# Nablax/Path-Tracer-CUDA-OpenGL

Measured on AMD Instinct MI355X. Metric: Mray/s + ms/frame, bunny-in-Cornell 1920×1080 @1024spp, 1/2/4/8 MI355X, higher is better.
Workload: dtype f32

## Files before the change

### path-tracer-cuda-opengl_amd/csrc/pt_device.hip

```cpp
#include <hip/hip_runtime.h>

#include <algorithm>
#include <array>
#include <atomic>
#include <chrono>
#include <cfloat>
#include <cmath>
#include <cstdio>
#include <cstdlib>
#include <cstring>
#include <limits>
#include <type_traits>
#include <memory>
#include <string>
#include <vector>

#include "../host/pt_error.hpp"
#include "../host/pt_host.hpp"
#include "../host/pt_inst_dev.hpp"
#include "../host/pt_wide8.hpp"
#include "../host/pt_wide_dev.hpp"
#include "pt.h"
#include "pt_math.hpp"

// ... 259 lines not shown
    float b1 = dot3(s1, s) * inv;
    float b2 = dot3(s2, d) * inv;
    if (b1 >= 1.0f || b1 <= 0.0f || b2 >= 1.0f || b2 <= 0.0f || b1 + b2 >= 1.0f || t <= tmin)
        return -1.0f;
    return t;
}

__device__ __forceinline__ SlabHit refLeafBox(const Prim& q, bool sphere, float3 o, float3 inv, float tmin, float tmax) {
    float mn[3], mx[3];
    if (sphere) {
        const float r = fabsf(q.p1.x);
        mn[0] = q.p0.x - r; mn[1] = q.p0.y - r; mn[2] = q.p0.z - r;
        mx[0] = q.p0.x + r; mx[1] = q.p0.y + r; mx[2] = q.p0.z + r;
    } else {
        mn[0] = fminf(fminf(q.p0.x, q.p1.x), q.p2.x);
        mn[1] = fminf(fminf(q.p0.y, q.p1.y), q.p2.y);
        mn[2] = fminf(fminf(q.p0.z, q.p1.z), q.p2.z);
        mx[0] = fmaxf(fmaxf(q.p0.x, q.p1.x), q.p2.x);
        mx[1] = fmaxf(fmaxf(q.p0.y, q.p1.y), q.p2.y);
        mx[2] = fmaxf(fmaxf(q.p0.z, q.p1.z), q.p2.z);
    }
    return slabPair(v2f{mn[0], mx[0]}, v2f{mn[1], mx[1]}, v2f{mn[2], mx[2]}, o, inv, tmin, tmax);
}

template <bool SPH>
__device__ __forceinline__ void wideTest(const Prim& q, float3 o, float3 d, float3 inv, float tmin, float& closest,
                                         int& best, float& bestLo, bool leafBoxes, bool& redo, uint32_t keyHi = 0u) {
    const bool sph = SPH && __float_as_uint(q.p2.w) != 0u;
    const float t = primHitAny(q, sph, o, d, tmin);
    if (t >= 0.0f) {
        const int k = (int)(keyHi | __float_as_uint(q.p0.w));
        const bool none = best < 0, bSph = SPH && (best & (int)kSphereBit) != 0;
        const int bk = SPH ? best & (int)kPrimMask : best;
        const bool tie = sph ? (none || !bSph || k > bk) : (!none && !bSph && k < bk);
        redo = redo || (t >= closest && t < bestLo);
        if (t < closest || (t == closest && tie)) {
            bool take = true;
            float lo = -__builtin_inff();
            if (leafBoxes) {
                const SlabHit b = refLeafBox(q, sph, o, inv, tmin, __builtin_inff());
                take = b.hit && !(closest < b.lo);
                redo = redo || (b.hit && closest < b.lo);
                lo = t < b.lo ? b.lo : lo;
            }
            if (take) {
                closest = t;
                best = k | (sph ? (int)kSphereBit : 0);
                bestLo = lo;
            }
        }
    }
}

__device__ __forceinline__ void wideTestTri(const Prim& q, float3 o, float3 d, float tmin, float& closest, int& best,
                                            float& t2) {
    const float t = primHitAny(q, false, o, d, tmin);
    if (t >= 0.0f) {
        const int k = (int)__float_as_uint(q.p0.w);
        const bool better = t < closest || (t == closest && k < best);
        t2 = __builtin_amdgcn_fmed3f(t, closest, t2);
        closest = better ? t : closest;
        best = better ? k : best;
    }
}
__device__ __forceinline__ bool deferredRedo(float4 xy, float2 z, float3 o, float3 inv, float closest, float t2) {
    const SlabHit b = slabPair(v2f{xy.x, xy.y}, v2f{xy.z, xy.w}, v2f{z.x, z.y}, o, inv, 0.001f, __builtin_inff());
    return !b.hit || (closest < b.lo && t2 < b.lo);
}

template <bool MIX = false>
__device__ __forceinline__ uint32_t wideHits(uint4 n0, uint4 n1, uint4 n2, uint4 n3, uint4 n4, float3 o, float3 inv,
                                             uint32_t oct, float tmin, float tmax) {
    constexpr uint32_t kMixExp = MIX ? 24u : 0u;
    const float ax = __uint_as_float(((n0.w & 0xffu) + kMixExp) << 23) * inv.x;
    const float ay = __uint_as_float((((n0.w >> 8) & 0xffu) + kMixExp) << 23) * inv.y;
    const float az = __uint_as_float((((n0.w >> 16) & 0xffu) + kMixExp) << 23) * inv.z;
    const float bx = (__uint_as_float(n0.x) - o.x) * inv.x;
    const float by = (__uint_as_float(n0.y) - o.y) * inv.y;
    const float bz = (__uint_as_float(n0.z) - o.z) * inv.z;
    const bool sx = (oct & 1u) != 0, sy = (oct & 2u) != 0, sz = (oct & 4u) != 0;
    const uint32_t nearX[2] = {sx ? n2.z : n2.x, sx ? n2.w : n2.y}, farX[2] = {sx ? n2.x : n2.z, sx ? n2.y : n2.w};
    const uint32_t nearY[2] = {sy ? n3.z : n3.x, sy ? n3.w : n3.y}, farY[2] = {sy ? n3.x : n3.z, sy ? n3.y : n3.w};
    const uint32_t nearZ[2] = {sz ? n4.z : n4.x, sz ? n4.w : n4.y}, farZ[2] = {sz ? n4.x : n4.z, sz ? n4.y : n4.w};
    const uint32_t oct2 = oct | shlOpaque<8>(oct);
    const uint32_t oct4 = oct2 | (oct2 << 16);
    uint32_t hits = 0u;
#pragma unroll
    for (int h = 0; h < 2; h++) {
        const uint32_t meta4 = h ? n1.w : n1.z;
        const uint32_t inner4 = (meta4 & (meta4 << 1)) & 0x10101010u;
        const uint32_t inner1 = inner4 >> 4;
        const uint32_t innerMask4 = shlOpaque<3>(inner1) - inner1;
        const uint32_t bitIndex4 = (meta4 ^ (oct4 & innerMask4)) & 0x1f1f1f1fu;
        const uint32_t childBits4 = (meta4 >> 5) & 0x07070707u;
#pragma unroll
        for (int j = 0; j < 4; j++) {
            float tnx, tny, tnz, tfx, tfy, tfz;
            if constexpr (MIX) {
                const bool hi = (j & 2) != 0;
                const uint32_t px = hi ? planePairHi(nearX[h]) : planePairLo(nearX[h]);
                const uint32_t py = hi ? planePairHi(nearY[h]) : planePairLo(nearY[h]);
                const uint32_t pz = hi ? planePairHi(nearZ[h]) : planePairLo(nearZ[h]);
                const uint32_t qx = hi ? planePairHi(farX[h]) : planePairLo(farX[h]);
                const uint32_t qy = hi ? planePairHi(farY[h]) : planePairLo(farY[h]);
                const uint32_t qz = hi ? planePairHi(farZ[h]) : planePairLo(farZ[h]);
                if (j & 1) {
                    tnx = fmaMixHi(px, ax, bx); tny = fmaMixHi(py, ay, by); tnz = fmaMixHi(pz, az, bz);
                    tfx = fmaMixHi(qx, ax, bx); tfy = fmaMixHi(qy, ay, by); tfz = fmaMixHi(qz, az, bz);
                } else {
                    tnx = fmaMixLo(px, ax, bx); tny = fmaMixLo(py, ay, by); tnz = fmaMixLo(pz, az, bz);
                    tfx = fmaMixLo(qx, ax, bx); tfy = fmaMixLo(qy, ay, by); tfz = fmaMixLo(qz, az, bz);
                }
            } else {
                tnx = __builtin_fmaf((float)((nearX[h] >> (8 * j)) & 0xffu), ax, bx);
                tny = __builtin_fmaf((float)((nearY[h] >> (8 * j)) & 0xffu), ay, by);
                tnz = __builtin_fmaf((float)((nearZ[h] >> (8 * j)) & 0xffu), az, bz);
// ... 737 lines not shown
        closest = __builtin_inff();                                                               \
        best = -1;                                                                                \
        sp = 0;                                                                                   \
        qn = 0;                                                                                   \
        if constexpr (CRITK) pxRays++;                                                            \
        if constexpr (WIDE) {                 \
            inv = f3(rcpRN(d.x), rcpRN(d.y), rcpRN(d.z));                                         \
            const uint32_t oc_ = (inv.x < 0.0f ? 1u : 0u) | (inv.y < 0.0f ? 2u : 0u) | (inv.z < 0.0f ? 4u : 0u); \
            oct = oc_;                                                                            \
            tg = 0u;                                                                              \
                    \
            bestLo = INST || kargs()->S.hasSpheres ? -__builtin_inff() : __builtin_inff();         \
            ng = S.nprims > 0 ? (1u << oc_) : 0u;                                                 \
                 \
            if (!INST && ((kargs()->camFar && depthLeft + 1 == kargs()->max_depth) ||              \
                          (PT_WIDE_MIX && mixUnsafe(inv, kargs()->S.mixLim)))) {                   \
                ng = 0u;             \
                oct |= 8u;      \
            }                                                                                     \
            if (INST && kargs()->camFar && depthLeft + 1 == kargs()->max_depth) {                  \
                     \
                const auto& K_ = *kargs();                                                        \
                (void)instEntry(K_.S.cx, K_.S.cy, K_.S.cz, K_.S.ext, o, d, inv);                   \
            }                                                                                     \
            if (CRITK && crit) PT_CRIT_TRACE();                                                    \
        } else if (S.nprims <= 1) {                                                               \
            node = -1;                                                                            \
            if (S.nprims == 1) {        \
                const float t1 = primHitT(loadPrim(S, 0), __float_as_uint(S.prims[2].w) != 0, o, d, \
                                          0.001f, closest);                                       \
                if (t1 >= 0.0f) { closest = t1; best = 0; }                                       \
            }                                                                                     \
        } else {                                                                                  \
            inv = f3(rcpRN(d.x), rcpRN(d.y), rcpRN(d.z));                                         \
            node = 0;                                                                             \
        }                                                                                         \
    } while (0)
#define PT_CRIT_TRACE()                                                                             \
    do {                                                                                          \
        const bool lb_ = S.nprims > 1;                                                            \
        const bool sph_ = kargs()->S.hasSpheres != 0;                                             \
        bool redo_ = false;                                                                       \
        for (;;) {                                                                                \
            while (tg) {                                                                          \
                const uint32_t k_ = tgBase + (uint32_t)__builtin_ctz(tg);                         \
                tg &= tg - 1u;                                                                    \
                const float4* w_ = reinterpret_cast<const float4*>(reinterpret_cast<const char*>(S.wprims) + mul48(k_)); \
                const Prim q_{w_[0], w_[1], w_[2]};                                               \
                const bool isS_ = __float_as_uint(q_.p2.w) != 0u;                                 \
                sTris += (uint32_t)__popcll(__ballot(!isS_));                                     \
                sSph += (uint32_t)__popcll(__ballot(isS_));                                       \
                if (sph_) wideTest<true>(q_, o, d, inv, 0.001f, closest, best, bestLo, lb_, redo_, 0u); \
                else if (INST) wideTest<false>(q_, o, d, inv, 0.001f, closest, best, bestLo, lb_, redo_, 0u); \
                else wideTestTri(q_, o, d, 0.001f, closest, best, bestLo);    \
            }                                                                                     \
            if ((ng & 0xffu) == 0u) {                                                             \
                if (sp == 0) break;                                                               \
                sp--;                                                                             \
                ng = my[sp * kWave];                                                              \
            }                                                                                     \
            const uint32_t bit_ = (uint32_t)__builtin_ctz(ng & 0xffu);                            \
            const uint32_t child_ = (ng >> 8) + (bit_ ^ (oct & 7u));                              \
            ng &= ~(1u << bit_);                                                                  \
            if (ng & 0xffu) { my[sp * kWave] = ng; sp++; }    \
            sVisits += (uint32_t)__popcll(__ballot(true));                                        \
            const uint32_t off_ = mul80(child_);                                                  \
            const uint4 n0_ = __builtin_bit_cast(uint4, __builtin_amdgcn_raw_buffer_load_b128(nodeRsrc, off_, 0, 0)); \
            const uint4 n1_ = __builtin_bit_cast(uint4, __builtin_amdgcn_raw_buffer_load_b128(nodeRsrc, off_ + 16u, 0, 0)); \
            const uint4 n2_ = __builtin_bit_cast(uint4, __builtin_amdgcn_raw_buffer_load_b128(nodeRsrc, off_ + 32u, 0, 0)); \
            const uint4 n3_ = __builtin_bit_cast(uint4, __builtin_amdgcn_raw_buffer_load_b128(nodeRsrc, off_ + 48u, 0, 0)); \
            const uint4 n4_ = __builtin_bit_cast(uint4, __builtin_amdgcn_raw_buffer_load_b128(nodeRsrc, off_ + 64u, 0, 0)); \
            const uint32_t h_ = wideHits<PT_WIDE_MIX != 0>(n0_, n1_, n2_, n3_, n4_, o, inv, oct & 7u, 0.001f, closest); \
            ng = (n1_.x << 8) | (h_ >> 24);                                                      \
            tgBase = n1_.y;                                                                       \
            tg = h_ & 0xffffffu;                                                                  \
        }                                                                                         \
        if (redo_) oct |= 8u;              \
    } while (0)
#define PT_TAKE_TASKS(got)                                                                          \
    do {                                                                                          \
        const auto& Q_ = *kargs();                                                                \
        for (;;) {                                                                                \
            const uint64_t m_ = needTaskM;                                                        \
            if (m_ == 0) break;                                                                   \
            if (poolLeft == 0u) {  \
                const int leader_ = __ffsll((unsigned long long)m_) - 1;                          \
                          \
                const uint32_t grab_ = (uint32_t)kTaskPool;                                       \
                uint32_t b_ = 0;                                                                  \
                if (lane == leader_) b_ = atomicAdd(Q_.taskCounter, grab_);                       \
                poolBase = __builtin_amdgcn_readfirstlane((uint32_t)__shfl((int)b_, leader_));    \
                poolLeft = grab_;                                                                 \
            }                                                                                     \
              \
            const uint32_t base_ = poolBase;                                                      \
            const uint32_t take_ = min((uint32_t)__popcll(m_), poolLeft);                         \
            poolBase += take_;                                                                    \
            poolLeft -= take_;                                                                    \
            const uint32_t g0_ = base_ >> 6, off_ = base_ & 63u;                                  \
            const uint32_t slotA_ = Q_.nblocksShift >= 0 ? g0_ >> Q_.nblocksShift : g0_ / (uint32_t)Q_.ngroups; \
            const uint32_t blkA_ = g0_ - slotA_ * (uint32_t)Q_.ngroups;                           \
            const bool wrap_ = blkA_ + 1u == (uint32_t)Q_.ngroups;                                  \
            const uint32_t slotB_ = wrap_ ? slotA_ + 1u : slotA_, blkB_ = wrap_ ? 0u : blkA_ + 1u; \
            const uint32_t nslots_ = (uint32_t)Q_.ntiles;                                          \
             \
                                                    \
            const uint32_t xyA_ = slotA_ < nslots_ ? ((KU32)Q_.tileXY)[__builtin_amdgcn_readfirstlane(slotA_)] : 0u; \
// ... 267 lines not shown
                        sp++;
                    }
                    node = (int)rref;
                } else if (il) {
                    node = (int)lref;
                } else if (sp > 0) {
                    sp--;
                    node = (LS == STACK || sp < LS)
                               ? (int)my[sp * kWave]
                               : (int)P.stackSpill[((size_t)blockIdx.x * kWave + lane) * (STACK - LS) + (sp - LS)];
                } else {
                    node = -1;
                }
            }
        }
        if (kind == 1) {
            bool tested = false, sph = false;
            PT_DIAG_ADD(itL, 1u);
            if constexpr (WIDE) {
                PT_DIAG_ADD(sPops, (uint32_t)nL);
                uint32_t k0 = 0u, k1 = 0u;
                const bool h0 = laneOf(mL);
                if (h0) k0 = tgBase + (uint32_t)__builtin_ctz(tg);
                tg &= tg - 1u;
                const uint64_t m1 = __ballot((int)tg > 0);
                const bool h1 = laneOf(m1);
                if (h1) k1 = tgBase + (uint32_t)__builtin_ctz(tg);
                tg &= tg - 1u;
                const float4* w0 = reinterpret_cast<const float4*>(reinterpret_cast<const char*>(S.wprims) + mul48(k0));
                const float4* w1 = reinterpret_cast<const float4*>(reinterpret_cast<const char*>(S.wprims) + mul48(k1));
                const Prim q0{w0[0], w0[1], w0[2]}, q1{w1[0], w1[1], w1[2]};
                bool redo = false;
#ifdef PT_DIAG
                {
                    sHalf += (unsigned long long)__popcll(__ballot(h0 && !h1));
                    const bool pk = !INST && (oct & 64u) != 0u;
                    sParkT += (unsigned long long)(__popcll(__ballot(pk && h0)) + __popcll(__ballot(pk && h1)));
                }
#endif
                const bool lb = !INST && S.nprims > 1;
                const uint32_t kh = INST ? (oct >> 8) << kargs()->S.gBits : 0u;
                if (kargs()->S.hasSpheres) {
                    if (h0) wideTest<true>(q0, o, d, inv, 0.001f, closest, best, bestLo, lb, redo, kh);
                    if (h1) wideTest<true>(q1, o, d, inv, 0.001f, closest, best, bestLo, lb, redo, kh);
                    const uint64_t s0 = mL & __ballot(__float_as_uint(q0.p2.w) != 0u);
                    const uint64_t s1 = m1 & __ballot(__float_as_uint(q1.p2.w) != 0u);
                    sTris += (uint32_t)nL + (uint32_t)__popcll(m1) - (uint32_t)__popcll(s0) - (uint32_t)__popcll(s1);
                    sSph += (uint32_t)__popcll(s0) + (uint32_t)__popcll(s1);
                } else {
                    if constexpr (INST) {
                        if (h0) wideTest<false>(q0, o, d, inv, 0.001f, closest, best, bestLo, lb, redo, kh);
                        if (h1) wideTest<false>(q1, o, d, inv, 0.001f, closest, best, bestLo, lb, redo, kh);
                    } else {
                        if (h0) wideTestTri(q0, o, d, 0.001f, closest, best, bestLo);
                        if (h1) wideTestTri(q1, o, d, 0.001f, closest, best, bestLo);
                    }
                    sTris += (uint32_t)nL + (uint32_t)__popcll(m1);
                }
                if (redo) oct |= 8u;
                if (SPEC && tg == 0u && (oct & 48u)) {
                    oct -= 16u;
                    const uint32_t c = SPECN == 1 ? 0u : (oct >> 4) & 3u;
                    tgBase = pend[(2u * c) * kWave + lane];
                    tg = pend[(2u * c + 1u) * kWave + lane];
#ifdef PT_DIAG
                    oct |= 64u;
#endif
                }
            } else {
            PT_DIAG_ADD(sPops, (uint32_t)nL);
            Prim pf0{}, pf1{};
            if (qn > 0) pf0 = loadPrim(S, qref[0] & kPrimMask);
            if (qn > 1) pf1 = loadPrim(S, qref[1] & kPrimMask);
#pragma unroll
            for (int k_ = 0; k_ < LQ; k_++) {
                const bool act = qn > 0;
                if (__ballot(act) == 0) break;
                tested = false;
                sph = false;
            if (act) {
                const uint32_t ref = qref[0];
                const float lo = lq[0];
#pragma unroll
                for (int i = 0; i + 1 < LQ; i++) { qref[i] = qref[i + 1]; lq[i] = lq[i + 1]; }
                qn--;
                const uint32_t k = ref & kPrimMask;
                sph = (ref & kSphereBit) != 0;
                if (!(closest < lo)) {
                    const Prim pr = k_ == 0 ? pf0 : (k_ == 1 ? pf1 : loadPrim(S, k));
                    {
                        tested = true;
                        const float t = primHitT(pr, sph, o, d, 0.001f, closest);
                        if (t >= 0.0f) { closest = t; best = (int)k; }
                    }
                }
            }
            sTris += (uint32_t)__popcll(__ballot(tested && !sph));
            sSph += (uint32_t)__popcll(__ballot(tested && sph));
            }
            }
        }
        if (kind == 2) {
            const uint64_t shadeM = mS & ~needTaskM;
            const bool shading = laneOf(shadeM);
            if constexpr (WIDE && !INST) {
                bool redo = shading && (oct & 8u);
#ifdef PT_DIAG
                bool missed = false;
// ... 1045 lines not shown
    explicit StreamGuard(hipStream_t s) : st(s) {}
    ~StreamGuard() {
        if (!ok) (void)hipStreamSynchronize(st);
        if (e0) (void)hipEventDestroy(e0);
        if (e1) (void)hipEventDestroy(e1);
    }
};

struct EventPair {
    hipEvent_t e0 = nullptr, e1 = nullptr;
    EventPair() = default;
    EventPair(const EventPair&) = delete;
    EventPair& operator=(const EventPair&) = delete;
    ~EventPair() {
        if (e0) (void)hipEventDestroy(e0);
        if (e1) (void)hipEventDestroy(e1);
    }
};
struct StreamWait {
    hipStream_t st;
    bool ok = false;
    explicit StreamWait(hipStream_t s) : st(s) {}
    ~StreamWait() {
        if (!ok) (void)hipStreamSynchronize(st);
    }
};

int stackFor(int depth) {
    const int need = depth + 1;
    for (int s : {16, 24, 32, 48, 64, 80})
        if (need <= s) return s;
    return -1;
}

struct InstEntry {
    uint32_t inst, mesh, slot;
};

}

struct pt_scene {
    int device = 0;
    int64_t nobj = 0, nmat = 0;
    bool hasSpheres = false;
    std::vector<pt_object> objs;
    DevBuf dobjs;
    DevBuf mats, nodes, prims, shade, counters;
    DevBuf keys, iparent, lparent, leafBoxes;
    DevBuf codes, ids, codes2, ids2, box6, sph, arr, dep, sortTemp;
    DevBuf irange;
    DevBuf refitEvents;
    DevBuf wide, wprims, wshade, rankOf;
    DevBuf wbox;
    std::unique_ptr<pt::WideDevBuilder> wideDev;
    bool wideReady = false;
    bool updated = false;
    int wideSource = 0;
    int wideDepth = 0;
    int64_t wideNodes = 0;
    double wideBuildMs = 0.0;
    int depth = 0;
    bool built = false;
    size_t deviceBytes = 0;
    double buildMs = 0.0;
    float sceneCE[4] = {0.0f, 0.0f, 0.0f, 0.0f};
    float skyH[3] = {1.0f, 1.0f, 1.0f}, skyZ[3] = {0.5f, 0.7f, 1.0f};
    bool hasEmissive = false;
    float mixLim = -1.0f;
    bool instanced = false;
    std::vector<int64_t> meshFirst, meshCount;
    std::vector<pt_instance> inst;
    DevBuf winst;
    int gBits = 0;
    bool instDynamic = false;
    bool instPrepared = false;
    std::vector<double> instReach;
    std::vector<InstEntry> instEntries;
    std::vector<uint32_t> instMeshRoot;
    uint32_t instTopCap = 0;
    int instMaxDepthB = 0;
    DevBuf instM, instDesc, instSub, instOut;
    DevBuf instPrims, instRank, instEntriesDev, instMeshRootDev, instWprims, instErr;
    EventPair instEvents;
    std::vector<float> instHostM;
    std::vector<double> instHostBox;
};

struct pt_film {
    int device = 0;
    int width = 0, height = 0, stripe_h = 1, nparts = 1, part = 0;
    int nrows = 0;
    int64_t npix = 0;
    uint64_t seed = 0;
    DevBuf state;
    DevBuf jumps;
    DevBuf tileCost, tileOrder;
    DevBuf tileXY, tileXYId;
    bool haveXYId = false;
    DevBuf tileKeys, tileKeys2, tileIds, sortTemp;
    bool haveOrder = false;
    int framesSinceCost = 0;
    DevBuf pixAcc, taskCounter;
    DevBuf pixRays, pixKeys, pixKeys2, pixIds, pixSorted, critFlag, critTemp;
    int critK = 0;
    DevBuf stackSpill;
    DevBuf sums;
    DevBuf accum;
    DevBuf staging;
    int64_t accumSamples = 0;
    int cus = 0;
    DevBuf counters;
    unsigned long long* hostCounters = nullptr;
    hipEvent_t ev0 = nullptr, ev1 = nullptr, ev2 = nullptr;
    bool rendered = false;
    bool lastWide = false;
    ~pt_film() {
        if (ev0) (void)hipEventDestroy(ev0);
        if (ev1) (void)hipEventDestroy(ev1);
        if (ev2) (void)hipEventDestroy(ev2);
        if (hostCounters) (void)hipHostFree(hostCounters);
    }
};

namespace {
int buildWide(pt_scene* s) {
    const int64_t n = s->nobj;
    std::vector<uint32_t> prims((size_t)n * pt::kW8PrimDwords), shade((size_t)n * 12);
    std::vector<float> boxes((size_t)n * 6);
    HIP_TRY(hipMemcpy(prims.data(), s->prims.p, prims.size() * 4, hipMemcpyDeviceToHost));
    HIP_TRY(hipMemcpy(shade.data(), s->shade.p, shade.size() * 4, hipMemcpyDeviceToHost));
    HIP_TRY(hipMemcpy(boxes.data(), s->leafBoxes.p, boxes.size() * 4, hipMemcpyDeviceToHost));
    std::vector<uint32_t> refs((size_t)std::max<int64_t>(1, n - 1) * 16);
    if (n > 1) HIP_TRY(hipMemcpy(refs.data(), s->nodes.p, (size_t)(n - 1) * 64, hipMemcpyDeviceToHost));
    const std::vector<uint32_t> rank = pt::referenceRanks(refs.data() + 12, refs.data() + 13, 16, n);
    std::vector<uint32_t> wshade(shade.size());
    for (int64_t k = 0; k < n; k++) std::memcpy(&wshade[(size_t)rank[k] * 12], &shade[(size_t)k * 12], 48);
    std::vector<float> wbox((size_t)n * pt::kW8BoxFloats);
    for (int64_t k = 0; k < n; k++)
        pt::exactTriBox(reinterpret_cast<const float*>(&prims[(size_t)k * pt::kW8PrimDwords]), &wbox[(size_t)rank[k] * pt::kW8BoxFloats]);
    pt::Wide8 w;
    std::string err;
    if (!pt::buildWide8(prims.data(), boxes.data(), rank.data(), n, w, err)) return fail(PT_ERR_STATE, err);
    int rc;
    if ((rc = devReserve(s->wide, w.nodes.size() * 4)) || (rc = devReserve(s->wprims, w.prims.size() * 4)) ||
        (rc = devReserve(s->wshade, wshade.size() * 4)) || (rc = devReserve(s->rankOf, rank.size() * 4)) ||
        (rc = devReserve(s->wbox, wbox.size() * 4)))
        return rc;
    HIP_TRY(hipMemcpy(s->wbox.p, wbox.data(), wbox.size() * 4, hipMemcpyHostToDevice));
    HIP_TRY(hipMemcpy(s->wide.p, w.nodes.data(), w.nodes.size() * 4, hipMemcpyHostToDevice));
    HIP_TRY(hipMemcpy(s->wprims.p, w.prims.data(), w.prims.size() * 4, hipMemcpyHostToDevice));
    HIP_TRY(hipMemcpy(s->wshade.p, wshade.data(), wshade.size() * 4, hipMemcpyHostToDevice));
    HIP_TRY(hipMemcpy(s->rankOf.p, rank.data(), rank.size() * 4, hipMemcpyHostToDevice));
    s->wideDepth = w.depth;
    s->wideNodes = (int64_t)(w.nodes.size() / pt::kW8NodeDwords);
    s->wideSource = 1;
    return PT_OK;
}

int buildWideDevice(pt_scene* s, hipStream_t st) {
    const int64_t n = s->nobj;
    int rc;
    if ((rc = devReserve(s->wide, (size_t)pt::wideDevNodeSlots(n) * pt::kW8NodeDwords * 4)) ||
        (rc = devReserve(s->wprims, (size_t)n * pt::kW8PrimDwords * 4)) || (rc = devReserve(s->wshade, (size_t)n * 48)) ||
        (rc = devReserve(s->rankOf, (size_t)n * 4)) || (rc = devReserve(s->wbox, (size_t)n * pt::kW8BoxFloats * 4)))
        return rc;
    if (!s->wideDev) s->wideDev.reset(new pt::WideDevBuilder);
    pt::WideDevIn in{s->prims.as<float4>(), s->shade.as<float4>(), s->leafBoxes.as<float>(), s->nodes.as<float4>(),
                     s->iparent.as<int>(), s->lparent.as<int>(), s->irange.as<int2>(), n};
    pt::WideDevOut out{s->wide.as<uint32_t>(), s->wprims.as<uint32_t>(), s->wshade.as<float4>(), s->wbox.as<float4>(),
                       s->rankOf.as<uint32_t>()};
    std::string err;
    const hipError_t e = s->wideDev->build(in, out, st, err);
    if (e != hipSuccess) return fail(err.empty() ? PT_ERR_HIP : PT_ERR_STATE, err.empty() ? hipGetErrorString(e) : err);
    s->wideDepth = out.depth;
    s->wideNodes = out.slots;
    s->wideSource = 2;
    return PT_OK;
}

int wideStackFor(int depth);
struct InstRecCtx {
    const std::vector<std::array<float, 12>>* minv;
    const std::vector<uint8_t>* ident;
    const std::vector<InstEntry>* entries;
};
uint32_t instanceOfRecord(const uint32_t* rec) { return rec[7]; }
void writeInstanceRecord(uint32_t e, uint32_t* dst, void* ctx) {
    const InstRecCtx& c = *static_cast<const InstRecCtx*>(ctx);
    const InstEntry& E = (*c.entries)[e];
    std::memset(dst, 0, pt::kW8NodeDwords * 4);
    dst[0] = (*c.ident)[E.inst] == 1 ? 1u : 0u;
    dst[1] = (*c.ident)[E.inst] == 2 ? 1u : 0u;
    dst[3] = pt::kW8InstanceFlag;
    dst[4] = E.slot;
    dst[5] = E.inst;
    dst[6] = E.mesh;
    std::memcpy(dst + 8, (*c.minv)[E.inst].data(), 48);
}

struct SubRoot {
    uint32_t slot;
    double box[6];
};
std::vector<SubRoot> nodeChildren(const pt::Wide8& w, uint32_t slot) {
    std::vector<SubRoot> out;
    if (w.nodes.size() < (size_t)(slot + 1) * pt::kW8NodeDwords) return out;
    const uint32_t* R = w.nodes.data() + (size_t)slot * pt::kW8NodeDwords;
    float p[3];
    std::memcpy(p, R, 12);
    for (int j = 0; j < 8; j++) {
        const uint32_t mb = (R[6 + (j >> 2)] >> (8 * (j & 3))) & 0xffu;
        if (mb == 0u) continue;
        if ((mb & 0xf8u) != 0x38u) return {};
        SubRoot sr;
        sr.slot = R[4] + (mb & 7u);
        for (int a = 0; a < 3; a++) {
            const int e = (int)((R[3] >> (8 * a)) & 0xffu) - 127;
            const uint32_t ql = (R[8 + 4 * a + (j >> 2)] >> (8 * (j & 3))) & 0xffu;
            const uint32_t qh = (R[10 + 4 * a + (j >> 2)] >> (8 * (j & 3))) & 0xffu;
            sr.box[a] = (double)p[a] + std::ldexp((double)ql, e);
            sr.box[3 + a] = (double)p[a] + std::ldexp((double)qh, e);
        }
        out.push_back(sr);
// ... 1266 lines not shown
              void* stream, pt_stats* stats) {
    return pt_render_ex(s, f, cam, spp, max_depth, out, on_dev, stream, nullptr, stats);
}

int pt_render_ex(pt_scene* s, pt_film* f, const pt_camera* cam, int spp, int max_depth, float* out, int on_dev,
                 void* stream, const pt_render_opts* opts, pt_stats* stats) {
    if (!s || !f || !cam || !out || spp <= 0) return fail(PT_ERR_INVALID, "pt_render: bad argument");
    if (!s->built) return fail(PT_ERR_STATE, "pt_render: BVH not built");
    if (s->device != f->device) return fail(PT_ERR_INVALID, "pt_render: scene and film on different devices");
    if (!(cam->lens_radius >= 0.0f) || !std::isfinite(cam->lens_radius))
        return fail(PT_ERR_INVALID, "pt_render: lens radius must be finite and >= 0");
    int rc = setDevice(s->device);
    if (rc) return rc;
    hipStream_t st = on_dev ? (hipStream_t)stream : 0;
    const int64_t np = f->npix;
    const int fmt = opts ? opts->out_format : PT_OUT_RGB32F;
    if (fmt != PT_OUT_RGB32F && fmt != PT_OUT_RGBA8 && fmt != PT_OUT_RGBA8_SURFACE)
        return fail(PT_ERR_INVALID, "pt_render_ex: unknown output format");
    const bool accumulate = opts && (opts->flags & PT_RENDER_ACCUMULATE);
    const size_t outBpp = fmt == PT_OUT_RGB32F ? 12 : 4;
    if (accumulate && f->accumSamples + spp >= (1ll << 24))
        return fail(PT_ERR_INVALID, "pt_render_ex: accumulated samples must stay below 2^24");
    int kernel = opts ? opts->kernel : PT_KERNEL_DEFAULT;
    if (kernel == PT_KERNEL_DEFAULT) {
        const char* k = std::getenv("PT_RENDER_KERNEL");
        const std::string ks = k ? k : "";
        kernel = ks == "simple" ? PT_KERNEL_SIMPLE : (ks == "wavefront" ? PT_KERNEL_WAVEFRONT : PT_KERNEL_WIDE);
    }
    if (kernel != PT_KERNEL_SIMPLE && kernel != PT_KERNEL_WAVEFRONT && kernel != PT_KERNEL_WIDE)
        return fail(PT_ERR_INVALID, "pt_render_ex: unknown kernel");
    if (s->instanced && kernel != PT_KERNEL_WIDE)
        return fail(PT_ERR_INVALID, "pt_render_ex: instanced scenes render with the wide kernel (PT_KERNEL_WIDE)");
    const int rng = opts ? opts->rng : PT_RNG_COMPAT;
    if (rng != PT_RNG_COMPAT && rng != PT_RNG_SAMPLE) return fail(PT_ERR_INVALID, "pt_render_ex: unknown rng mode");
    if (kernel == PT_KERNEL_WIDE && (rc = ensureWide(s))) return rc;

    if (!f->ev0) {
        HIP_TRY(hipEventCreate(&f->ev0));
        HIP_TRY(hipEventCreate(&f->ev1));
        HIP_TRY(hipEventCreateWithFlags(&f->ev2, hipEventDisableTiming));
    }
    if (!f->counters.p && (rc = devAlloc(f->counters, kNumCounters * sizeof(unsigned long long)))) return rc;
    if (!f->hostCounters) HIP_TRY(hipHostMalloc(reinterpret_cast<void**>(&f->hostCounters),
                                                kNumCounters * sizeof(unsigned long long), hipHostMallocDefault));
    void* dst = out;
    if (!on_dev) {
        if ((rc = devReserve(f->staging, (size_t)std::max<int64_t>(1, np) * outBpp))) return rc;
        dst = f->staging.p;
    }
    HIP_TRY(hipMemsetAsync(f->counters.p, 0, kNumCounters * sizeof(unsigned long long), st));
    RenderParams P;
    P.S = devScene(s);
    P.S.err = reinterpret_cast<unsigned int*>(f->counters.as<unsigned long long>() + 7);
    P.cam.pos = make_float3(cam->origin[0], cam->origin[1], cam->origin[2]);
    P.cam.ll = make_float3(cam->lower_left[0], cam->lower_left[1], cam->lower_left[2]);
    P.cam.hor = make_float3(cam->horizontal[0], cam->horizontal[1], cam->horizontal[2]);
    P.cam.ver = make_float3(cam->vertical[0], cam->vertical[1], cam->vertical[2]);
    P.cam.right = make_float3(cam->right[0], cam->right[1], cam->right[2]);
    P.cam.up = make_float3(cam->up[0], cam->up[1], cam->up[2]);
    P.cam.lens = cam->lens_radius;
    P.skyH = make_float3(s->skyH[0], s->skyH[1], s->skyH[2]);
    P.skyZ = make_float3(s->skyZ[0], s->skyZ[1], s->skyZ[2]);
    {
        static const float H0[3] = {1.0f, 1.0f, 1.0f}, Z0[3] = {0.5f, 0.7f, 1.0f};
        P.lit = (s->hasEmissive || std::memcmp(s->skyH, H0, sizeof(H0)) != 0 || std::memcmp(s->skyZ, Z0, sizeof(Z0)) != 0) ? 1 : 0;
    }
    uint32_t* b = f->state.as<uint32_t>();
    P.sd = b; P.s0 = b + np; P.s1 = b + 2 * np; P.s2 = b + 3 * np; P.s3 = b + 4 * np; P.s4 = b + 5 * np;
    P.out = static_cast<float*>(dst);
    P.rawOut = 0;
    P.sampleBase = 0;
    P.counters = f->counters.as<unsigned long long>();
    P.width = f->width;
    P.nrows = f->nrows;
    P.stripe_h = f->stripe_h;
    P.stripeShift = (f->stripe_h & (f->stripe_h - 1)) == 0 ? __builtin_ctz((unsigned)f->stripe_h) : -1;
    P.nparts = f->nparts;
    P.part = f->part;
    P.tiles_x = (f->width + 7) / 8;
    P.ntiles = P.tiles_x * ((f->nrows + 7) / 8);
    P.spp = spp;
    P.max_depth = max_depth;
    P.invW = 1.0f / (float)f->width;
    P.invH = 1.0f / (float)f->height;
    P.invSpp = 1.0f / (float)spp;
    if (kernel == PT_KERNEL_WIDE && s->nobj > 0 && (!P.S.wnodes || !P.S.wprims)) return fail(PT_ERR_STATE, "wide BVH missing");
    P.kernel = kernel;
    P.nblocks = 0;
    P.block = 0;
    P.blockShift = -1;
    P.group = 1;
    P.span = 0;
    P.ngroups = 0;
    P.pixAcc = nullptr;
    P.taskCounter = nullptr;
    P.stackSpill = nullptr;
    P.ntasks = 0;
    P.nwaves = 0;
    P.seed0 = (uint32_t)f->seed;
    P.seed1 = (uint32_t)(f->seed >> 32);
    P.measureCost = 0;
    {
        double m = 0.0;
        for (int a = 0; a < 3; a++)
            m = std::max(m, std::fabs((double)cam->origin[a] - (double)s->sceneCE[a]) +
                                (double)cam->lens_radius * (std::fabs((double)cam->right[a]) + std::fabs((double)cam->up[a])));
// ... 258 lines not shown
```

### path-tracer-cuda-opengl_amd/csrc/pt_wide_build.hip

```cpp
#include <hip/hip_runtime.h>

#include <cmath>
#include <cstdlib>
#include <cstring>

#include "pt_prims.hpp"
#include "pt_wide8.hpp"
#include "pt_wide_dev.hpp"

namespace pt {
namespace {

constexpr uint32_t kRefLeaf = 0x80000000u, kRefMask = 0x3fffffffu;
constexpr uint32_t kGroupFlag = 0x80000000u;
constexpr int kRadiusDefault = 8;
constexpr int kTile = 256;
constexpr int kMaxGroup = 3;
constexpr int kMaxLevels = 24;
enum { kMiscNodes = 0, kMiscM = 1, kMiscTotA = 3, kMiscTotB = 4, kMiscTotC = 5, kMiscErr = 6, kMiscWords = 8 };
constexpr int kPassesPerSync = 4;

__device__ __forceinline__ float areaOf(float4 lo, float4 hi) {
    const float dx = hi.x - lo.x, dy = hi.y - lo.y, dz = hi.z - lo.z;
    return dx * dy + dy * dz + dz * dx;
}
__device__ __forceinline__ float4 minBox(float4 a, float4 b) { return make_float4(fminf(a.x, b.x), fminf(a.y, b.y), fminf(a.z, b.z), 0.0f); }
__device__ __forceinline__ float4 maxBox(float4 a, float4 b) { return make_float4(fmaxf(a.x, b.x), fmaxf(a.y, b.y), fmaxf(a.z, b.z), 0.0f); }

__device__ __forceinline__ int ceilLog2(double x) {
    int e = 0;
    const double m = frexp(x, &e);
    return m == 0.5 ? e - 1 : e;
}

__global__ void rankKernel(const float4* __restrict__ lbvh, const int* __restrict__ iparent,
                           const int* __restrict__ lparent, const int2* __restrict__ irange, int n, uint32_t* rank) {
    const int k = blockIdx.x * blockDim.x + threadIdx.x;
    if (k >= n) return;
    uint32_t r = 0;
    int child = k, p = lparent[k];
    bool leaf = true;
    for (int guard = 0; p >= 0 && guard < 130; guard++) {
        const float4 refs = lbvh[4 * (size_t)p + 3];
        const uint32_t lref = __float_as_uint(refs.x), rref = __float_as_uint(refs.y);
        const bool lLeaf = lref & kRefLeaf, rLeaf = rref & kRefLeaf;
        const bool isLeft = leaf ? (lLeaf && (int)(lref & kRefMask) == child) : (!lLeaf && (int)lref == child);
        const uint32_t nl = (lLeaf ? 1u : 0u) + (rLeaf ? 1u : 0u);
        if (leaf) r += (!isLeft && lLeaf) ? 1u : 0u;
        else if (!isLeft) r += nl;
        else r += nl + (rLeaf ? 0u : (uint32_t)(irange[rref].y - irange[rref].x + 1));
        child = p;
        leaf = false;
        p = iparent[p];
    }
    rank[k] = r;
}

__global__ void shadeByRankKernel(const float4* __restrict__ shade, const float4* __restrict__ prims,
                                  const uint32_t* __restrict__ rank, int n, float4* wshade, float4* wbox) {
    const int k = blockIdx.x * blockDim.x + threadIdx.x;
    if (k >= n) return;
    const size_t r = rank[k];
    wshade[3 * r] = shade[3 * (size_t)k];
    wshade[3 * r + 1] = shade[3 * (size_t)k + 1];
    wshade[3 * r + 2] = shade[3 * (size_t)k + 2];
    const float4 a = prims[3 * (size_t)k], b = prims[3 * (size_t)k + 1], c = prims[3 * (size_t)k + 2];
    wbox[2 * r] = make_float4(fminf(fminf(a.x, b.x), c.x), fmaxf(fmaxf(a.x, b.x), c.x), fminf(fminf(a.y, b.y), c.y),
                              fmaxf(fmaxf(a.y, b.y), c.y));
    wbox[2 * r + 1] = make_float4(fminf(fminf(a.z, b.z), c.z), fmaxf(fmaxf(a.z, b.z), c.z), 0.0f, 0.0f);
}

__global__ void plocInitKernel(const float* __restrict__ leafBoxes, int n, float4* pbox, uint32_t* cid) {
    const int k = blockIdx.x * blockDim.x + threadIdx.x;
    if (k >= n) return;
    const float* b = leafBoxes + 6 * (size_t)k;
    const float4 lo = make_float4(b[0], b[1], b[2], 0.0f), hi = make_float4(b[3], b[4], b[5], 0.0f);
    pbox[2 * (size_t)k] = make_float4(lo.x, lo.y, lo.z, areaOf(lo, hi));
    pbox[2 * (size_t)k + 1] = make_float4(hi.x, hi.y, hi.z, __uint_as_float(1u));
    cid[k] = (uint32_t)k;
}

template <int kRadius>
__global__ __launch_bounds__(kTile) void plocNearestKernel(const uint32_t* __restrict__ cid, const float4* __restrict__ pbox,
                                                           const uint32_t* __restrict__ mDev, int* nn) {
    const int m = (int)*mDev;
    __shared__ float4 tlo[kTile + 2 * kRadius], thi[kTile + 2 * kRadius];
    const int base = blockIdx.x * kTile - kRadius;
    for (int t = threadIdx.x; t < kTile + 2 * kRadius; t += kTile) {
        const int j = base + t;
        if (j >= 0 && j < m) {
            const size_t id = cid[j];
            tlo[t] = pbox[2 * id];
            thi[t] = pbox[2 * id + 1];
        }
    }
    __syncthreads();
    const int i = blockIdx.x * kTile + threadIdx.x;
    if (i >= m) return;
    const int ti = threadIdx.x + kRadius;
    const float4 lo = tlo[ti], hi = thi[ti];
    int best = -1;
    float bestA = INFINITY;
    uint64_t bestKey = ~0ull;
    for (int o = -kRadius; o <= kRadius; o++) {
        const int j = i + o;
        if (o == 0 || j < 0 || j >= m) continue;
        const float a = areaOf(minBox(lo, tlo[ti + o]), maxBox(hi, thi[ti + o]));
        const int mn = o < 0 ? j : i;
        const uint64_t key = ((uint64_t)(o < 0 ? -o : o) << 27) | ((uint64_t)(mn & 1) << 26) | (uint64_t)mn;
        if (a < bestA || (a == bestA && key < bestKey)) {
            bestA = a;
            bestKey = key;
            best = j;
        }
    }
    nn[i] = best;
}

__device__ __forceinline__ void makeNode(float4* pbox, uint2* pchild, uint32_t n, uint32_t id, uint32_t a, uint32_t b,
                                         float kTravCost) {
    const float4 la = pbox[2 * (size_t)a], ha = pbox[2 * (size_t)a + 1];
    const float4 lb = pbox[2 * (size_t)b], hb = pbox[2 * (size_t)b + 1];
// ... 1290 lines not shown
        WB_TRY(hipGetLastError());
        int64_t m = n;
        {
            const uint32_t m0 = (uint32_t)n;
            WB_TRY(hipMemcpyAsync(misc + kMiscM, &m0, 4, hipMemcpyHostToDevice, st));
        }
        int pass = 0;
        while (m > kTailMax) {
            if (pass > 4 * 64 + 64) {
                err = "wide BVH (device): clustering does not converge";
                return hipErrorUnknown;
            }
            for (int b = 0; b < kPassesPerSync; b++, pass++) {
                uint32_t* cid = static_cast<uint32_t*>(cid_[cur].p);
                const uint32_t* mIn = misc + kMiscM + (pass & 1);
                switch (radius) {
                    case 8: plocNearestKernel<8><<<blocks(m, kTile), kTile, 0, st>>>(cid, pbox, mIn, nearest); break;
                    case 32: plocNearestKernel<32><<<blocks(m, kTile), kTile, 0, st>>>(cid, pbox, mIn, nearest); break;
                    case 64: plocNearestKernel<64><<<blocks(m, kTile), kTile, 0, st>>>(cid, pbox, mIn, nearest); break;
                    default: plocNearestKernel<16><<<blocks(m, kTile), kTile, 0, st>>>(cid, pbox, mIn, nearest); break;
                }
                plocMergeKernel<<<blocks(m, tb), tb, 0, st>>>(cid, pbox, pchild, nearest, mIn, (int)m, (int)n, trav, flag, misc);
                WB_TRY(hipGetLastError());
                WB_TRY(exclusiveScanU32(scanTemp_.p, flag, pos, (size_t)m, st));
                plocCompactKernel<<<blocks(m, tb), tb, 0, st>>>(cid, flag, pos, mIn, static_cast<uint32_t*>(cid_[cur ^ 1].p),
                                                                misc + kMiscM + ((pass + 1) & 1));
                WB_TRY(hipGetLastError());
                cur ^= 1;
            }
            uint32_t mNext = 0;
            WB_TRY(hipMemcpyAsync(&mNext, misc + kMiscM + (pass & 1), 4, hipMemcpyDeviceToHost, st));
            WB_TRY(hipStreamSynchronize(st));
            if ((int64_t)mNext >= m) {
                err = "wide BVH (device): clustering passes merged nothing";
                return hipErrorUnknown;
            }
            m = mNext;
        }
        if (m > 1) {
            uint32_t* a0 = static_cast<uint32_t*>(cid_[cur].p);
            uint32_t* a1 = static_cast<uint32_t*>(cid_[cur ^ 1].p);
            const uint32_t* mIn = misc + kMiscM + (pass & 1);
            switch (radius) {
                case 8: plocTailKernel<8><<<1, kTailThreads, 0, st>>>(a0, a1, pbox, pchild, nearest, flag, mIn, misc, (int)n, trav); break;
                case 32: plocTailKernel<32><<<1, kTailThreads, 0, st>>>(a0, a1, pbox, pchild, nearest, flag, mIn, misc, (int)n, trav); break;
                case 64: plocTailKernel<64><<<1, kTailThreads, 0, st>>>(a0, a1, pbox, pchild, nearest, flag, mIn, misc, (int)n, trav); break;
                default: plocTailKernel<16><<<1, kTailThreads, 0, st>>>(a0, a1, pbox, pchild, nearest, flag, mIn, misc, (int)n, trav); break;
            }
            WB_TRY(hipGetLastError());
        }
    }
    const uint32_t* rootCid = static_cast<const uint32_t*>(cid_[cur].p);

    return collapseLevels(n, rootCid, wideDevSlotCap(n) , 0u, in.prims,
                          out.rank, out.nodes, out.wprims, st, err, out.depth, out.slots);
}

}
```

### path-tracer-cuda-opengl_amd/host/pt_wide8.hpp

```cpp
#pragma once
#include <cmath>
#include <cstdint>
#include <string>
#include <vector>

namespace pt {

#ifndef PT_NODE_DWORDS
#define PT_NODE_DWORDS 20
#endif
constexpr int kW8NodeDwords = PT_NODE_DWORDS;
static_assert(kW8NodeDwords == 20 || kW8NodeDwords == 32, "node slots of 80 or 128 B");
constexpr int kW8PrimDwords = 12;
constexpr int kW8BoxFloats = 8;

inline void exactTriBox(const float* rec, float* out) {
    for (int a = 0; a < 3; a++) {
        out[2 * a] = std::fmin(std::fmin(rec[a], rec[4 + a]), rec[8 + a]);
        out[2 * a + 1] = std::fmax(std::fmax(rec[a], rec[4 + a]), rec[8 + a]);
    }
    out[6] = out[7] = 0.0f;
}

#ifndef PT_WIDE_EMIN_SHIFT
#define PT_WIDE_EMIN_SHIFT 18
#endif
#ifndef PT_WIDE_FAR_EXT
#define PT_WIDE_FAR_EXT 8.0f
#endif
constexpr int kW8EminShift = PT_WIDE_EMIN_SHIFT;
constexpr float kW8FarExt = PT_WIDE_FAR_EXT;
static_assert(kW8EminShift >= 0 && kW8EminShift < 31 &&
                  (double)kW8FarExt * (double)(1u << kW8EminShift) <= 8.0 * (double)(1u << 18),
              "PT_WIDE_EMIN_SHIFT and PT_WIDE_FAR_EXT move together: far line * 2^shift <= 8 * 2^18");

struct Wide8 {
    std::vector<uint32_t> nodes;
    std::vector<uint32_t> prims;
    int depth = 0;
    int64_t usedNodes = 0;
    int64_t leaves = 0;
};

bool buildWide8(const uint32_t* prims, const float* boxes, const uint32_t* rank, int64_t n, Wide8& out,
                std::string& err, double scaleFloor = 0.0);
bool buildWide8Leaf(const uint32_t* prims, const float* boxes, const uint32_t* rank, int64_t n, int maxLeaf,
                    Wide8& out, std::string& err, double scaleFloor = 0.0);

constexpr uint32_t kW8InstanceFlag = 0xff000000u;
void relocateWide8(Wide8& w, uint32_t nodeBase, uint32_t primBase);
bool instanceLeaves(Wide8& top, uint32_t (*instanceOf)(const uint32_t* primRecord),
                    void (*record)(uint32_t id, uint32_t* dst, void* ctx), void* ctx, std::string& err);

std::vector<uint32_t> referenceRanks(const uint32_t* leftRef, const uint32_t* rightRef, size_t stride, int64_t n);

}
```

### path-tracer-cuda-opengl_amd/host/pt_wide_dev.hpp

```cpp
#pragma once
#include <hip/hip_runtime.h>

#include <cstdint>
#include <string>

namespace pt {

struct WideDevIn {
    const float4* prims;
    const float4* shade;
    const float* leafBoxes;
    const float4* lbvh;
    const int* iparent;
    const int* lparent;
    const int2* irange;
    int64_t n;
};

struct WideDevOut {
    uint32_t* nodes;
    uint32_t* wprims;
    float4* wshade;
    float4* wbox;
    uint32_t* rank;
    int depth = 0;
    int64_t slots = 0;
};

inline int64_t wideDevNodeSlots(int64_t n) { return 1 + 8 * ((n > 1 ? n - 1 : 0) / 7 + 1); }
constexpr int64_t kWideMaxSlots = (int64_t)1 << 24;
inline uint32_t wideDevSlotCap(int64_t n) {
    const int64_t s = wideDevNodeSlots(n);
    return (uint32_t)(s < kWideMaxSlots ? s : kWideMaxSlots);
}

class WideDevBuilder {
public:
    WideDevBuilder() = default;
    WideDevBuilder(const WideDevBuilder&) = delete;
    WideDevBuilder& operator=(const WideDevBuilder&) = delete;
    ~WideDevBuilder();
    hipError_t build(const WideDevIn& in, WideDevOut& out, hipStream_t stream, std::string& err);
    hipError_t reserveTop(int64_t n);
    hipError_t buildTop(const float* leafBoxes, int64_t n, const float4* prims, const uint32_t* rank, uint32_t* nodes,
                        uint32_t* wprims, uint32_t slotCap, hipStream_t stream, std::string& err, int& depth, int64_t& slots);

private:
    struct Buf {
        void* p = nullptr;
        size_t cap = 0;
    };
    hipError_t reserve(Buf& b, size_t bytes);
    hipError_t buildSah(const WideDevIn& in, hipStream_t stream, float trav, int maxGroup, std::string& err);
    hipError_t reserveScratch(int64_t n);
    hipError_t reserveSah(int64_t n);
    hipError_t collapseLevels(int64_t n, const uint32_t* rootCid, uint32_t slotCap, uint32_t everyBlock, const float4* prims,
                              const uint32_t* rank, uint32_t* nodes, uint32_t* wprims, hipStream_t stream, std::string& err,
                              int& depth, int64_t& slots);
    Buf pbox_, pchild_, cid_[2], nn_, flag_, pos_, items_[2], cnt_, ofs_, scanTemp_, misc_;
    Buf sahCen_, sahRef_[2], sahLarge_[2], sahSmall_, sahSplit_, sahBins_, sahMulti_, sahBlk_, sahBlkR_, sahBlkO_, sahCnt_;
};

}
```

Measured before the change: 21850.

## Precompute triangle edge records and use wave-ballot Möller–Trumbore test

Adds a parallel triangle record buffer that stores v0 plus precomputed edges e1 and e2, built both on the host and via a new device kernel after the wide BVH collapse. In triangle-only, non-instanced scenes the renderer points wprims at this buffer. The triangle test is rewritten as an inline Möller–Trumbore using a fast Newton reciprocal with a wave-level fallback and ballot masks, replacing per-lane branches on h0/h1. The aim is to cut per-hit subtractions and divergence. The cost is extra memory and build work, and every lane in the wave now computes each test even when masked out.

Result: faster. 22340, median of 6 (+2.3%).

```diff
diff --git a/path-tracer-cuda-opengl_amd/csrc/pt_device.hip b/path-tracer-cuda-opengl_amd/csrc/pt_device.hip
--- a/path-tracer-cuda-opengl_amd/csrc/pt_device.hip
+++ b/path-tracer-cuda-opengl_amd/csrc/pt_device.hip
@@ -335,16 +335,34 @@
     }
 }
 
-__device__ __forceinline__ void wideTestTri(const Prim& q, float3 o, float3 d, float tmin, float& closest, int& best,
-                                            float& t2) {
-    const float t = primHitAny(q, false, o, d, tmin);
-    if (t >= 0.0f) {
-        const int k = (int)__float_as_uint(q.p0.w);
-        const bool better = t < closest || (t == closest && k < best);
-        t2 = __builtin_amdgcn_fmed3f(t, closest, t2);
-        closest = better ? t : closest;
-        best = better ? k : best;
-    }
+__device__ __forceinline__ float rcpRNWave(float x, uint64_t hasM) {
+    if constexpr (!PT_FAST_RCP) return 1.0f / x;
+    const uint32_t ex = (__float_as_uint(x) >> 23) & 0xffu;
+    const uint64_t slowM = hasM & __ballot(ex - kRcpExpLo > kRcpExpHi - kRcpExpLo);
+    float y = rcpNewton(x);
+    if (__builtin_expect(slowM != 0, 0)) y = __builtin_amdgcn_inverse_ballot_w64(slowM) ? 1.0f / x : y;
+    return y;
+}
+__device__ __forceinline__ void wideTestTri(const Prim& q, uint64_t hasM, float3 o, float3 d, float tmin, float& closest,
+                                            int& best, float& t2) {
+    const float3 v0 = xyz(q.p0), e1 = xyz(q.p1), e2 = xyz(q.p2);
+    const float3 s1 = cross3(d, e2);
+    const float det = dot3(s1, e1);
+    const float3 s = sub(o, v0);
+    const float3 s2 = cross3(s, e1);
+    const float inv = rcpRNWave(det, hasM);
+    const float t = dot3(s2, e2) * inv;
+    const float b1 = dot3(s1, s) * inv;
+    const float b2 = dot3(s2, d) * inv;
+    const int k = (int)__float_as_uint(q.p0.w);
+    const uint64_t rejM = __ballot(b1 >= 1.0f) | __ballot(b1 <= 0.0f) | __ballot(b2 >= 1.0f) | __ballot(b2 <= 0.0f) |
+                          __ballot(b1 + b2 >= 1.0f);
+    const uint64_t hitM = hasM & __ballot(det != 0.0f) & __ballot(t > tmin) & ~rejM;
+    const uint64_t takeM = hitM & (__ballot(t < closest) | (__ballot(t == closest) & __ballot(k < best)));
+    const float mid = __builtin_amdgcn_fmed3f(t, closest, t2);
+    t2 = __builtin_amdgcn_inverse_ballot_w64(hitM) ? mid : t2;
+    closest = __builtin_amdgcn_inverse_ballot_w64(takeM) ? t : closest;
+    best = __builtin_amdgcn_inverse_ballot_w64(takeM) ? k : best;
 }
 __device__ __forceinline__ bool deferredRedo(float4 xy, float2 z, float3 o, float3 inv, float closest, float t2) {
     const SlabHit b = slabPair(v2f{xy.x, xy.y}, v2f{xy.z, xy.w}, v2f{z.x, z.y}, o, inv, 0.001f, __builtin_inff());
@@ -1188,7 +1206,7 @@
                 sSph += (uint32_t)__popcll(__ballot(isS_));                                       \
                 if (sph_) wideTest<true>(q_, o, d, inv, 0.001f, closest, best, bestLo, lb_, redo_, 0u); \
                 else if (INST) wideTest<false>(q_, o, d, inv, 0.001f, closest, best, bestLo, lb_, redo_, 0u); \
-                else wideTestTri(q_, o, d, 0.001f, closest, best, bestLo);    \
+                else wideTestTri(q_, __ballot(true), o, d, 0.001f, closest, best, bestLo);    \
             }                                                                                     \
             if ((ng & 0xffu) == 0u) {                                                             \
                 if (sp == 0) break;                                                               \
@@ -1562,8 +1580,8 @@
                         if (h0) wideTest<false>(q0, o, d, inv, 0.001f, closest, best, bestLo, lb, redo, kh);
                         if (h1) wideTest<false>(q1, o, d, inv, 0.001f, closest, best, bestLo, lb, redo, kh);
                     } else {
-                        if (h0) wideTestTri(q0, o, d, 0.001f, closest, best, bestLo);
-                        if (h1) wideTestTri(q1, o, d, 0.001f, closest, best, bestLo);
+                        wideTestTri(q0, mL, o, d, 0.001f, closest, best, bestLo);
+                        wideTestTri(q1, m1, o, d, 0.001f, closest, best, bestLo);
                     }
                     sTris += (uint32_t)nL + (uint32_t)__popcll(m1);
                 }
@@ -2715,6 +2733,8 @@
     DevBuf refitEvents;
     DevBuf wide, wprims, wshade, rankOf;
     DevBuf wbox;
+    DevBuf wtris;
+    bool haveWtris = false;
     std::unique_ptr<pt::WideDevBuilder> wideDev;
     bool wideReady = false;
     bool updated = false;
@@ -2805,6 +2825,13 @@
     std::string err;
     if (!pt::buildWide8(prims.data(), boxes.data(), rank.data(), n, w, err)) return fail(PT_ERR_STATE, err);
     int rc;
+    s->haveWtris = !s->hasSpheres;
+    if (s->haveWtris) {
+        std::vector<uint32_t> wtris(w.prims.size());
+        pt::edgeTriRecords(w.prims.data(), n, wtris.data());
+        if ((rc = devReserve(s->wtris, wtris.size() * 4))) return rc;
+        HIP_TRY(hipMemcpy(s->wtris.p, wtris.data(), wtris.size() * 4, hipMemcpyHostToDevice));
+    }
     if ((rc = devReserve(s->wide, w.nodes.size() * 4)) || (rc = devReserve(s->wprims, w.prims.size() * 4)) ||
         (rc = devReserve(s->wshade, wshade.size() * 4)) || (rc = devReserve(s->rankOf, rank.size() * 4)) ||
         (rc = devReserve(s->wbox, wbox.size() * 4)))
@@ -2827,11 +2854,13 @@
         (rc = devReserve(s->wprims, (size_t)n * pt::kW8PrimDwords * 4)) || (rc = devReserve(s->wshade, (size_t)n * 48)) ||
         (rc = devReserve(s->rankOf, (size_t)n * 4)) || (rc = devReserve(s->wbox, (size_t)n * pt::kW8BoxFloats * 4)))
         return rc;
+    s->haveWtris = !s->hasSpheres;
+    if (s->haveWtris && (rc = devReserve(s->wtris, (size_t)n * pt::kW8PrimDwords * 4))) return rc;
     if (!s->wideDev) s->wideDev.reset(new pt::WideDevBuilder);
     pt::WideDevIn in{s->prims.as<float4>(), s->shade.as<float4>(), s->leafBoxes.as<float>(), s->nodes.as<float4>(),
                      s->iparent.as<int>(), s->lparent.as<int>(), s->irange.as<int2>(), n};
     pt::WideDevOut out{s->wide.as<uint32_t>(), s->wprims.as<uint32_t>(), s->wshade.as<float4>(), s->wbox.as<float4>(),
-                       s->rankOf.as<uint32_t>()};
+                       s->rankOf.as<uint32_t>(), s->haveWtris ? s->wtris.as<uint32_t>() : nullptr};
     std::string err;
     const hipError_t e = s->wideDev->build(in, out, st, err);
     if (e != hipSuccess) return fail(err.empty() ? PT_ERR_HIP : PT_ERR_STATE, err.empty() ? hipGetErrorString(e) : err);
@@ -4204,6 +4233,7 @@
     RenderParams P;
     P.S = devScene(s);
     P.S.err = reinterpret_cast<unsigned int*>(f->counters.as<unsigned long long>() + 7);
+    if (s->wideReady && s->haveWtris && !s->hasSpheres && !s->instanced) P.S.wprims = s->wtris.as<float4>();
     P.cam.pos = make_float3(cam->origin[0], cam->origin[1], cam->origin[2]);
     P.cam.ll = make_float3(cam->lower_left[0], cam->lower_left[1], cam->lower_left[2]);
     P.cam.hor = make_float3(cam->horizontal[0], cam->horizontal[1], cam->horizontal[2]);
diff --git a/path-tracer-cuda-opengl_amd/csrc/pt_wide_build.hip b/path-tracer-cuda-opengl_amd/csrc/pt_wide_build.hip
--- a/path-tracer-cuda-opengl_amd/csrc/pt_wide_build.hip
+++ b/path-tracer-cuda-opengl_amd/csrc/pt_wide_build.hip
@@ -68,6 +68,18 @@
     wbox[2 * r] = make_float4(fminf(fminf(a.x, b.x), c.x), fmaxf(fmaxf(a.x, b.x), c.x), fminf(fminf(a.y, b.y), c.y),
                               fmaxf(fmaxf(a.y, b.y), c.y));
     wbox[2 * r + 1] = make_float4(fminf(fminf(a.z, b.z), c.z), fmaxf(fmaxf(a.z, b.z), c.z), 0.0f, 0.0f);
+}
+
+__global__ void edgeRecordsKernel(const uint4* __restrict__ wprims, int n, uint4* __restrict__ wtris) {
+    const int k = blockIdx.x * blockDim.x + threadIdx.x;
+    if (k >= n) return;
+    const uint4 a = wprims[3 * (size_t)k], b = wprims[3 * (size_t)k + 1], c = wprims[3 * (size_t)k + 2];
+    const float ax = __uint_as_float(a.x), ay = __uint_as_float(a.y), az = __uint_as_float(a.z);
+    wtris[3 * (size_t)k] = a;
+    wtris[3 * (size_t)k + 1] = make_uint4(__float_as_uint(__uint_as_float(b.x) - ax), __float_as_uint(__uint_as_float(b.y) - ay),
+                                          __float_as_uint(__uint_as_float(b.z) - az), b.w);
+    wtris[3 * (size_t)k + 2] = make_uint4(__float_as_uint(__uint_as_float(c.x) - ax), __float_as_uint(__uint_as_float(c.y) - ay),
+                                          __float_as_uint(__uint_as_float(c.z) - az), c.w);
 }
 
 __global__ void plocInitKernel(const float* __restrict__ leafBoxes, int n, float4* pbox, uint32_t* cid) {
@@ -1464,8 +1476,14 @@
     }
     const uint32_t* rootCid = static_cast<const uint32_t*>(cid_[cur].p);
 
-    return collapseLevels(n, rootCid, wideDevSlotCap(n) , 0u, in.prims,
-                          out.rank, out.nodes, out.wprims, st, err, out.depth, out.slots);
-}
-
-}
+    WB_TRY(collapseLevels(n, rootCid, wideDevSlotCap(n) , 0u, in.prims,
+                          out.rank, out.nodes, out.wprims, st, err, out.depth, out.slots));
+    if (out.wtris) {
+        edgeRecordsKernel<<<blocks(n, tb), tb, 0, st>>>(reinterpret_cast<const uint4*>(out.wprims), (int)n,
+                                                        reinterpret_cast<uint4*>(out.wtris));
+        WB_TRY(hipGetLastError());
+    }
+    return hipSuccess;
+}
+
+}
diff --git a/path-tracer-cuda-opengl_amd/host/pt_wide8.hpp b/path-tracer-cuda-opengl_amd/host/pt_wide8.hpp
--- a/path-tracer-cuda-opengl_amd/host/pt_wide8.hpp
+++ b/path-tracer-cuda-opengl_amd/host/pt_wide8.hpp
@@ -1,6 +1,7 @@
 #pragma once
 #include <cmath>
 #include <cstdint>
+#include <cstring>
 #include <string>
 #include <vector>
 
@@ -20,6 +21,21 @@
         out[2 * a + 1] = std::fmax(std::fmax(rec[a], rec[4 + a]), rec[8 + a]);
     }
     out[6] = out[7] = 0.0f;
+}
+
+inline void edgeTriRecords(const uint32_t* prims, int64_t n, uint32_t* out) {
+    for (int64_t k = 0; k < n; k++) {
+        const uint32_t* src = prims + (size_t)k * kW8PrimDwords;
+        uint32_t* dst = out + (size_t)k * kW8PrimDwords;
+        float v[kW8PrimDwords];
+        std::memcpy(v, src, sizeof(v));
+        std::memcpy(dst, src, sizeof(v));
+        for (int a = 0; a < 3; a++) {
+            const float e1 = v[4 + a] - v[a], e2 = v[8 + a] - v[a];
+            std::memcpy(dst + 4 + a, &e1, 4);
+            std::memcpy(dst + 8 + a, &e2, 4);
+        }
+    }
 }
 
 #ifndef PT_WIDE_EMIN_SHIFT
diff --git a/path-tracer-cuda-opengl_amd/host/pt_wide_dev.hpp b/path-tracer-cuda-opengl_amd/host/pt_wide_dev.hpp
--- a/path-tracer-cuda-opengl_amd/host/pt_wide_dev.hpp
+++ b/path-tracer-cuda-opengl_amd/host/pt_wide_dev.hpp
@@ -23,6 +23,7 @@
     float4* wshade;
     float4* wbox;
     uint32_t* rank;
+    uint32_t* wtris = nullptr;
     int depth = 0;
     int64_t slots = 0;
 };
```
